# utiasSTARS/GraphIK

Measured on AMD Instinct MI355X. Metric: IK solves/sec (batched random goals), higher is better.
Workload: dtype f64

## Files before the change

graphik_amd/_ffi.py:

```python
import ctypes as C
import os

import torch

_HERE = os.path.dirname(os.path.abspath(__file__))
LIB_PATH = os.environ.get("GIK_LIB_PATH") or os.path.join(_HERE, "lib", "libgraphik_amd.so")

TERM_EQ, TERM_LOWER, TERM_UPPER = 1, 2, 3
ABI_VERSION = 10


class TemplateDesc(C.Structure):
    _fields_ = [
        ("abi_version", C.c_int32), ("N", C.c_int32), ("k", C.c_int32), ("n_terms", C.c_int32),
        ("term_i", C.POINTER(C.c_int32)), ("term_j", C.POINTER(C.c_int32)),
        ("term_kind", C.POINTER(C.c_int32)),
        ("mingradnorm", C.c_double), ("maxiter", C.c_int32), ("maxinner", C.c_int32),
        ("mininner", C.c_int32), ("theta", C.c_double), ("kappa", C.c_double),
        ("rho_prime", C.c_double), ("rho_regularization", C.c_double),
        ("planar_proj_exact", C.c_int32), ("force_block_path", C.c_int32),
        ("waves_per_cu", C.c_int32), ("slice_outer_its", C.c_int32), ("debug_flags", C.c_int32),
        ("solver", C.c_int32), ("cg_minstepsize", C.c_double), ("cg_orth_value", C.c_double),
        ("cg_beta_type", C.c_int32), ("clique_closed_form", C.c_int32), ("hessian_form", C.c_int32),
    ]


CLIQUE_AUTO, CLIQUE_OFF, CLIQUE_DENSE = 0, 1, 2
HESS_COLUMN, HESS_PER_EDGE, HESS_AUTO = 0, 1, 2


class TemplateInfo(C.Structure):
    _fields_ = [("is_block", C.c_int32), ("max_terms_per_node", C.c_int32), ("n_clique", C.c_int32),
                ("n_slot_terms", C.c_int32), ("slots_per_thread", C.c_int32), ("waves_per_cu", C.c_int32),
                ("n_cu", C.c_int32), ("lds_bytes", C.c_int32), ("clique_closed_form", C.c_int32),
                ("anchored", C.c_int32), ("has_pipeline", C.c_int32), ("prepare_is_block", C.c_int32),
                ("node_per_lane", C.c_int32), ("problems_per_wave", C.c_int32), ("goals_per_wave", C.c_int32),
                ("hessian_form", C.c_int32)]


SOLVER_TRUST_REGIONS, SOLVER_CONJUGATE_GRADIENT = 0, 1


class Stats(C.Structure):
    _fields_ = [("f", C.c_double), ("gradnorm", C.c_double), ("iterations", C.c_int32),
                ("inner_total", C.c_int32), ("stop", C.c_int32), ("n_accept", C.c_int32),
                ("inner_executed", C.c_int32), ("flags", C.c_int32), ("stepsize", C.c_double)]


STATS_BYTES = C.sizeof(Stats)
STATS_I32 = {name: getattr(Stats, name).offset // 4 for name, ct in Stats._fields_ if ct is C.c_int32}
STATS_F64 = {name: getattr(Stats, name).offset // 8 for name, ct in Stats._fields_ if ct is C.c_double}


class Trace(C.Structure):
    _fields_ = [("cap", C.c_int32), ("d_Delta", C.c_void_p), ("d_numit", C.c_void_p),
                ("d_stop", C.c_void_p), ("d_f_before", C.c_void_p),
                ("d_gradnorm_after", C.c_void_p), ("d_accept", C.c_void_p)]


class PipelineDesc(C.Structure):
# ... 65 lines not shown
                                        C.c_void_p, C.c_void_p, C.c_void_p, C.c_void_p, C.c_void_p]),
    "gik_anchored_seed_batch": (C.c_int, [C.c_void_p, C.c_void_p, C.c_void_p, C.c_void_p, C.c_int, C.c_void_p,
                                          C.c_void_p, C.c_void_p, C.c_void_p]),
    "gik_anchored_clearance": (C.c_int, [C.c_void_p, C.c_void_p, C.c_int, C.c_void_p, C.c_void_p]),
    "gik_anchored_attach_links": (C.c_int, [C.c_void_p, C.POINTER(LinkDesc)]),
    "gik_anchored_link_clearance": (C.c_int, [C.c_void_p, C.c_void_p, C.c_int, C.c_void_p, C.c_void_p]),
    "gik_anchored_sweep_ws_bytes": (C.c_size_t, [C.c_void_p, C.c_void_p, C.c_int, C.c_int]),
    "gik_anchored_sweep_clearance": (C.c_int, [C.c_void_p, C.c_void_p, C.c_void_p, C.c_void_p, C.c_int, C.c_int, C.c_void_p,
                                               C.c_void_p, C.c_void_p]),
    "gik_anchored_ik_batch_seeded": (C.c_int, [C.c_void_p, C.c_void_p, C.c_void_p, C.c_void_p, C.c_int] +
                                     7 * [C.c_void_p] + [C.c_void_p]),
    "gik_anchored_last_solve_ms": (C.c_double, [C.c_void_p]),
    "gik_anchored_retry_select": (C.c_int, [C.c_void_p, C.c_void_p, C.c_void_p, C.c_void_p, C.c_int, C.c_double,
                                            C.c_double, C.c_double, C.c_void_p, C.c_void_p, C.c_void_p]),
    "gik_anchored_retry_seeds": (C.c_int, [C.c_void_p, C.c_void_p, C.c_void_p, C.c_int, C.c_uint64, C.c_int, C.c_void_p,
                                           C.c_void_p, C.c_void_p, C.c_double, C.c_void_p, C.c_void_p, C.c_void_p]),
    "gik_anchored_retry_merge": (C.c_int, [C.c_void_p, C.c_void_p, C.c_void_p, C.c_int, C.c_int, C.c_double, C.c_double,
                                           C.c_double] + 13 * [C.c_void_p] + [C.c_void_p]),
    "gik_anchored_retry_ws_bytes": (C.c_size_t, [C.c_void_p, C.c_void_p, C.c_int]),
    "gik_anchored_ik_batch_retry": (C.c_int, [C.c_void_p, C.c_void_p, C.c_void_p, C.c_void_p, C.c_int,
                                              C.POINTER(AnchoredRetryOpts)] + 8 * [C.c_void_p] + [C.c_void_p]),
    "gik_template_destroy": (None, [C.c_void_p]),
    "gik_template_get_info": (C.c_int, [C.c_void_p, C.POINTER(TemplateInfo)]),
    "gik_cost": (C.c_int, [C.c_void_p, C.c_void_p, C.c_void_p, C.c_int, C.c_void_p, C.c_void_p]),
    "gik_grad": (C.c_int, [C.c_void_p, C.c_void_p, C.c_void_p, C.c_int, C.c_void_p, C.c_void_p]),
    "gik_cost_and_grad": (C.c_int, [C.c_void_p, C.c_void_p, C.c_void_p, C.c_int, C.c_void_p, C.c_void_p,
                                    C.c_void_p]),
    "gik_hess": (C.c_int, [C.c_void_p, C.c_void_p, C.c_void_p, C.c_void_p, C.c_int, C.c_void_p,
                           C.c_void_p]),
    "gik_proj": (C.c_int, [C.c_void_p, C.c_void_p, C.c_void_p, C.c_int, C.c_void_p, C.c_void_p]),
    "gik_solve_batch": (C.c_int, [C.c_void_p, C.c_void_p, C.c_void_p, C.c_int, C.c_void_p,
                                  C.c_void_p, C.POINTER(Trace), C.c_void_p]),
    "gik_pipeline_attach": (C.c_int, [C.c_void_p, C.POINTER(PipelineDesc)]),
    "gik_prepare_batch": (C.c_int, [C.c_void_p, C.c_void_p, C.c_int, C.c_void_p, C.c_void_p,
                                    C.c_void_p, C.c_void_p]),
    "gik_prepare_batch_debug": (C.c_int, [C.c_void_p, C.c_void_p, C.c_int, C.c_void_p, C.c_void_p,
                                          C.c_void_p, C.POINTER(PrepareDiag), C.c_void_p]),
    "gik_recover_batch": (C.c_int, [C.c_void_p, C.c_void_p, C.c_void_p, C.c_int, C.c_void_p,
                                    C.c_void_p, C.c_void_p, C.c_void_p]),
    "gik_ik_batch": (C.c_int, [C.c_void_p, C.c_void_p, C.c_int, C.c_void_p, C.c_void_p,
                               C.c_void_p, C.c_void_p, C.c_void_p, C.c_void_p, C.c_void_p]),
    "gik_seed_batch": (C.c_int, [C.c_void_p, C.c_void_p, C.c_void_p, C.c_int, C.c_void_p, C.c_void_p,
                                 C.c_void_p]),
    "gik_ik_batch_seeded": (C.c_int, [C.c_void_p, C.c_void_p, C.c_void_p, C.c_int, C.c_void_p, C.c_void_p,
                                      C.c_void_p, C.c_void_p, C.c_void_p, C.c_void_p, C.c_void_p]),
    "gik_retry_select": (C.c_int, [C.c_void_p, C.c_void_p, C.c_void_p, C.c_int, C.c_double, C.c_double,
# ... 54 lines not shown
```

graphik_amd/build.py:

```python
import glob
import hashlib
import os
import shutil
import subprocess
import sys

HERE = os.path.dirname(os.path.abspath(__file__))
REPO = os.path.dirname(HERE)
SRC = os.path.join(HERE, "csrc")
LIB = os.path.join(HERE, "lib", "libgraphik_amd.so")
DEV_LIB = os.path.join(HERE, "lib", "exp", "libgraphik_amd_dev.so")
SOURCES = ["gik_host.hip", "gik_k_wave3.hip", "gik_k_wave3_strict.hip", "gik_k_anch.hip", "gik_k_wave2.hip",
           "gik_k_block.hip", "gik_k_npt.hip", "gik_k_npt4.hip", "gik_k_quad.hip", "gik_k_prep.hip", "gik_k_retry.hip", "gik_k_anch_seed.hip",
           "gik_k_anch_retry.hip"]
FLAGS = ["--offload-arch=gfx950", "-O3", "-std=c++17", "-fPIC"]
LINK_FLAGS = ["--offload-arch=gfx950", "-shared", "-fPIC"]
UNIT_FLAGS = {"gik_k_wave3_strict.hip": ["-mllvm", "-structurizecfg-skip-uniform-regions"]}


def headers():
    return sorted(glob.glob(os.path.join(SRC, "*.h")) + glob.glob(os.path.join(REPO, "include", "*.h")))


def dependencies():
    deps = sorted(glob.glob(os.path.join(SRC, "*.hip")) + headers())
    assert all(os.path.join(SRC, s) in deps for s in SOURCES)
    return deps


def source_digest(extra=()):
    h = hashlib.sha256(" ".join(FLAGS + LINK_FLAGS + list(extra)).encode())
    h.update(repr(sorted(UNIT_FLAGS.items())).encode())
    for d in dependencies():
        h.update(os.path.relpath(d, REPO).encode())
        h.update(open(d, "rb").read())
    return h.hexdigest()

# ... 90 lines not shown
```

graphik_amd/csrc/gik_host.hip:

```cpp

#include "gik_kernels.hip.h"
#include "gik_instances.h"
#include "gik_retry.hip.h"
#include "gik_anch_seed.hip.h"
#include "gik_anch_retry.hip.h"
#include "gik_plan.h"
#include "gik_slots.h"
#include <climits>
#include <memory>

namespace gik {
GIK_ALL_KERNELS(GIK_EXTERN_TEMPLATE)
static_assert(PLAN_MIG_SIMDS == MIG_SIMDS && PLAN_SLICE_STATE_BYTES == sizeof(SliceState) && PLAN_QUAD_SLOTS == QUAD_SLOTS,
              "gik_plan.h restates these constants of the kernel headers");

struct NptVariant {
  int TL, NW;
  void (*solve)(SolveArgs);
  void (*kat)(KatArgs);
  size_t (*lds)(int, int, int, int);
  size_t (*ctg)(int);
};
#define GIK_NPT_VARIANT(TL, NS, NW, CTG) \
  {TL, NW, rtr_npt_kernel<TL, NS, NW, CTG>, kat_npt_kernel<TL, NS, NW, CTG>, NptCtx<TL, NS, NW, CTG>::lds_bytes, NptCtx<TL, NS, NW, CTG>::ctg_doubles}
static const NptVariant kNptVariants[] = {GIK_NPT_VARIANT(1, 1, 2, false), GIK_NPT_VARIANT(4, 1, 2, false),
                                          GIK_NPT_VARIANT(1, 2, 1, false), GIK_NPT_VARIANT(4, 2, 1, false),
                                          GIK_NPT_VARIANT(1, 1, 4, true),  GIK_NPT_VARIANT(4, 1, 4, true)};

thread_local std::string g_err;
#ifdef GIK_DEV
static double *g_dbg_buf = nullptr;
#endif
static int fail(const std::string &m) {
  g_err = m;
  return -1;
}
#define HIP_OK(expr)                                                                      \
// ... 69 lines not shown
  hipEvent_t ev_solve0 = nullptr, ev_solve1 = nullptr;
  gik::AnchArgs an = {};
  double *d_targets_const = nullptr;
  int full_N = 0, n_anchor = 0;
  int *d_free_full = nullptr, *d_anchor_full = nullptr;
  int *d_clear_full = nullptr;
  int n_clear = 0;
  int *d_link_a = nullptr, *d_link_b = nullptr;
  double *d_link_rho = nullptr;
  int n_link = -1;
  double axis_length = 1.0;
  int solver;
  gik::CgParams cg;
  gik::Params p;
  struct Kernels {
    void (*solve)(gik::SolveArgs) = nullptr;
    void (*solve_spread)(gik::SolveArgs) = nullptr;
    void (*kat)(gik::KatArgs) = nullptr;
    void (*block_solve)(gik::SolveArgs, int) = nullptr;
    void (*block_kat)(gik::KatArgs, int) = nullptr;
    const void *occupancy = nullptr;
  } kernels;
  uint32_t *d_slot_meta = nullptr;
  unsigned int *d_counters = nullptr;
  struct CounterSlot {
    hipEvent_t done = nullptr;
    bool pending = false;
    bool in_use = false;
  };
  std::vector<CounterSlot> counter_slot;
  unsigned next_counter = 0;
  int counter_ring = 256;
  std::mutex call_mutex;
  std::mutex ev_mutex;
  int clique_mode = 0;
  bool hess_per_edge = false;
  struct SliceWs {
    void *base = nullptr;
    size_t bytes = 0;
    hipEvent_t done = nullptr;
    bool pending = false;
    bool in_use = false;
  };
  static constexpr int kSlicePool = 32;
  SliceWs slice_ws[kSlicePool];
  unsigned next_slice = 0;
// ... 1865 lines not shown
  a.slot_meta = t->d_slot_meta;
  a.bt = t->bt;
  a.targets = d_targets;
  a.Y_init = d_Y_init;
  a.Y_out = d_Y_out;
  a.stats = d_stats;
  a.has_trace = (trace && trace->cap > 0) ? 1 : 0;
  if (a.has_trace)
    a.trace = *trace;
  else
    std::memset(&a.trace, 0, sizeof(a.trace));
  a.N = t->N;
  a.T = t->T;
  a.B = B;
  a.p = t->p;
  a.cg = t->cg;
  if (t->anchored) {
    a.an = t->an;
    a.an.anchor_goal = d_targets;
    a.targets = t->d_targets_const;
  }
  a.dbg = t->f.dbg;
  a.dbg_buf = nullptr;
#ifdef GIK_DEV
  if (a.dbg & (4 | 8 | 4096)) a.dbg_buf = dev_debug_buffer();
#endif
  a.y_head = a.y_tail = a.y_seq = nullptr;
  a.y_ids = a.y_avail = nullptr;
  a.y_cap = 0;
  a.q_tail = a.q_done = a.q_head = nullptr;
  a.mig_credits = a.mig_simd_run = nullptr;
  a.q_ids = nullptr;
  a.q_seq = nullptr;
  a.q_state = nullptr;
}

static bool event_done(hipEvent_t e) {
  if (hipEventQuery(e) == hipSuccess) return true;
  (void)hipGetLastError();
  return false;
}

typedef gik::SlotLease<gik_template::CounterSlot> CounterLease;
typedef gik::SlotLease<gik_template::SliceWs> WorkspaceLease;

static int lease_counter(gik_template *mt, CounterLease &lease, gik::SolveArgs &a, hipStream_t stream) {
  using namespace gik;
  gik_template::CounterSlot &cs = lease.take(mt->counter_slot, mt->next_counter, (unsigned)mt->counter_ring, event_done);
  a.work_counter = mt->d_counters + (&cs - mt->counter_slot.data());
  if (!cs.done && hipEventCreateWithFlags(&cs.done, hipEventDisableTiming) != hipSuccess)
    return fail("hipEventCreate failed");
  if (cs.pending) HIP_OK(hipStreamWaitEvent(stream, cs.done, 0));
  HIP_OK(hipMemsetAsync(a.work_counter, 0, sizeof(unsigned int), stream));
  return 0;
}

static int bind_workspace(gik_template *mt, WorkspaceLease &lease, const gik::SolvePlan &p, gik::SolveArgs &a,
                          hipStream_t stream) {
  using namespace gik;
  gik_template::SliceWs *sw = &lease.take(mt->slice_ws, mt->next_slice, (unsigned)mt->slice_pool, event_done);
  if (!sw->done && hipEventCreateWithFlags(&sw->done, hipEventDisableTiming) != hipSuccess)
    return fail("hipEventCreate failed");
  if (sw->bytes < p.bytes) {
    if (sw->pending) (void)hipEventSynchronize(sw->done);
    if (sw->base) (void)hipFree(sw->base);
    sw->base = nullptr;
    sw->bytes = 0;
    if (hipMalloc(&sw->base, p.bytes) != hipSuccess) return fail("cannot allocate the time-slicing workspace");
    sw->bytes = p.bytes;
    sw->pending = false;
  }
  if (sw->pending) HIP_OK(hipStreamWaitEvent(stream, sw->done, 0));
  char *base = static_cast<char *>(sw->base);
  a.q_tail = reinterpret_cast<unsigned int *>(base);
  a.q_done = a.q_tail + 1;
  a.q_head = a.q_tail + 2;
  a.mig_credits = reinterpret_cast<int *>(a.q_tail + 3);
  a.mig_simd_run = reinterpret_cast<int *>(base + p.off_simd);
  a.q_seq = reinterpret_cast<unsigned int *>(base + p.off_seq);
  a.q_ids = reinterpret_cast<int *>(base + p.off_ids);
  a.q_state = reinterpret_cast<SliceState *>(base + p.off_state);
  a.y_head = a.q_tail + 4;
  a.y_tail = a.q_tail + 5;
  a.y_avail = reinterpret_cast<int *>(a.q_tail + 6);
  a.y_seq = reinterpret_cast<unsigned int *>(base + p.off_yseq);
  a.y_ids = reinterpret_cast<int *>(base + p.off_yids);
  a.y_cap = (unsigned int)p.ycap;
  a.npt_ctg_ws = p.ctg_bytes ? reinterpret_cast<double *>(base + p.off_ctg) : nullptr;
  HIP_OK(hipMemsetAsync(base, 0, p.zero_head, stream));
  if (p.seq_fill) HIP_OK(hipMemsetAsync(a.q_seq, 0xFF, p.seq_fill, stream));
  if (p.state_zero) HIP_OK(hipMemsetAsync(a.q_state, 0, p.state_zero, stream));
  if (p.yseq_zero) HIP_OK(hipMemsetAsync(a.y_seq, 0, p.yseq_zero, stream));
  return 0;
}

static void launch(const gik_template *t, const gik::SolvePlan &p, gik::SolveArgs &a, hipStream_t stream) {
  using namespace gik;
  const dim3 grid(p.launch_grid);
  switch (p.launch) {
    case Launch::QUAD:
      hipLaunchKernelGGL(t->quad_solve, grid, dim3(WAVE), t->quad_smem, stream, a);
      break;
    case Launch::NPT:
      a.nt = t->nt;
      hipLaunchKernelGGL(t->npt_variant->solve, grid, dim3(WAVE * t->npt_variant->NW), t->npt_smem, stream, a);
      break;
    case Launch::BLOCK:
      hipLaunchKernelGGL(t->kernels.block_solve, grid, dim3(BLOCK_NT), t->smem_bytes, stream, a, t->SL);
      break;
    case Launch::WAVE:
      hipLaunchKernelGGL(t->kernels.solve, grid, dim3(WAVE), t->smem_bytes, stream, a);
      break;
    case Launch::WAVE_SPREAD:
      hipLaunchKernelGGL(t->kernels.solve_spread, grid, dim3(WAVE), t->smem_bytes, stream, a);
      break;
// ... 12 lines not shown
  fill_args(t, a, d_Y_init, d_targets, B, d_Y_out, d_stats, trace);
  if (refuse_capture("gik_solve_batch", stream_)) return -1;
  const SolvePlan plan = plan_solve(t->f, B);
  a.slice_its = plan.slice_its;
  a.slice_cycles = plan.slice_cycles;
  gik_template *mt = const_cast<gik_template *>(t);
  CounterLease counter(mt->call_mutex);
  WorkspaceLease workspace(mt->call_mutex);
  if (lease_counter(mt, counter, a, stream)) return -1;
  if (plan.needs_ws && bind_workspace(mt, workspace, plan, a, stream)) return -1;
  launch(t, plan, a, stream);
  HIP_OK(hipGetLastError());
  const hipError_t e_cs = hipEventRecord(counter.get()->done, stream);
  const hipError_t e_sw = workspace.get() ? hipEventRecord(workspace.get()->done, stream) : hipSuccess;
  if (e_cs != hipSuccess || e_sw != hipSuccess) {
    (void)hipStreamSynchronize(stream);
    return fail(std::string("hipEventRecord failed after the launch: ") + hipGetErrorString(e_cs != hipSuccess ? e_cs : e_sw));
  }
  counter.covered_by_event();
  workspace.covered_by_event();
  return 0;
}

int gik_template_get_info(const gik_template *t, gik_template_info *info) {
  if (!t || !info) return gik::fail("null argument");
  std::memset(info, 0, sizeof(*info));
  info->is_block = t->f.is_block ? 1 : 0;
  info->max_terms_per_node = t->f.is_block ? 0 : t->maxdeg;
  info->n_clique = t->bt.n_clq;
  info->n_slot_terms = t->f.is_block ? t->bt.Tc : t->T;
  info->slots_per_thread = t->SL;
  info->waves_per_cu = t->f.waves_per_cu;
  info->n_cu = t->f.n_cu;
  info->lds_bytes = (int32_t)t->smem_bytes;
  info->clique_closed_form = t->clique_mode;
  info->hessian_form = (t->hess_per_edge || t->f.is_block) ? GIK_HESS_PER_EDGE : GIK_HESS_COLUMN;
  info->anchored = t->anchored ? 1 : 0;
  info->has_pipeline = t->has_pipe ? 1 : 0;
  info->prepare_is_block = t->prep_block ? 1 : 0;
  info->node_per_lane = t->f.is_npt ? t->npt_variant->NW : 0;
  info->goals_per_wave = !t->has_pipe || t->prep_block ? 0 : (t->prep_quad ? gik::QUAD_SLOTS : 1);
  info->problems_per_wave = t->f.is_block ? 0 : ((t->quad_solve && !(t->f.dbg & (1 | 8192))) ? gik::QUAD_SLOTS : 1);
  if (t->f.is_npt) {
    info->waves_per_cu = t->f.npt_waves_per_cu;
    info->lds_bytes = (int32_t)t->npt_smem;
  }
  return 0;
}

#ifdef GIK_DEV
double gik_debug_parts(const gik_template *t, int mode, int iters) {
  using namespace gik;
  double *d = nullptr, h[2] = {0, 0};
  if (hipMalloc((void **)&d, 2 * sizeof(double)) != hipSuccess) return -1;
  hipEvent_t e0, e1;
  (void)hipEventCreate(&e0);
  (void)hipEventCreate(&e1);
  (void)hipEventRecord(e0, 0);
  if (t->f.K == 3 && t->maxdeg == 9)
    hipLaunchKernelGGL((parts_kernel<3, 9>), dim3(1), dim3(WAVE), t->smem_bytes, 0, t->d_slot_meta,
                       t->N, t->T, mode % 100, iters, d);
  else if (t->f.K == 3 && t->maxdeg == 10)
    hipLaunchKernelGGL((parts_kernel<3, 10>), dim3(1), dim3(WAVE), t->smem_bytes, 0, t->d_slot_meta,
                       t->N, t->T, mode % 100, iters, d);
// ... 22 lines not shown
```

graphik_amd/csrc/gik_kernels.hip.h:

```cpp
#pragma once
#include <hip/hip_runtime.h>

#include <algorithm>
#include <atomic>
#include <cmath>
#include <cstdio>
#include <cstring>
#include <mutex>
#include <thread>
#include <cstdlib>
#include <string>
#include <vector>

#include "gik_block.hip.h"
#include "gik_npt.hip.h"
#include "gik_quad.hip.h"
#include "gik_prep.hip.h"
#include "gik_prep_quad.hip.h"
#include "gik_rcg.hip.h"
#include "gik_rtr.hip.h"
#include "gik_rtrv.hip.h"
#include "gik_wave.hip.h"
#ifdef GIK_STRICT_HEADER
#include GIK_STRICT_HEADER
// ... 46 lines not shown
__device__ inline void requeue_work(unsigned int *q_tail, int *q_ids, unsigned int *q_seq, int B, int b) {
  const unsigned int t = atomicAdd(q_tail, 1u);
  __hip_atomic_store(&q_ids[t], b, __ATOMIC_RELAXED, __HIP_MEMORY_SCOPE_AGENT);
  __hip_atomic_store(&q_seq[t], (unsigned)B + t, __ATOMIC_RELEASE, __HIP_MEMORY_SCOPE_AGENT);
}

struct AnchArgs {
  const double *anch_const;
  const double *anchor_goal;
  const uint32_t *pin_meta;
  const double *pin_tgt;
  const double *obs;
  unsigned long long obs_mask;
  int n_obs, n_goal, goal_row0;
};

struct SolveArgs {
  const uint32_t *slot_meta;
  const double *targets;
  const double *Y_init;
  double *Y_out;
  gik_stats *stats;
  unsigned int *work_counter;
  gik_trace trace;
  int has_trace;
  int N, T, B;
  int dbg;
  double *dbg_buf;
  Params p;
  CgParams cg;
  AnchArgs an;
  int slice_its;
  int slice_cycles;
  unsigned int *q_head;
  int *mig_credits, *mig_simd_run;
  unsigned int *y_head, *y_tail, *y_seq;
  int *y_ids, *y_avail;
  unsigned int y_cap;
  unsigned int *q_tail, *q_done;
  int *q_ids;
  unsigned int *q_seq;
  SliceState *q_state;
  BlockTabs bt;
  NptTabs nt;
  double *npt_ctg_ws = nullptr;
};
// ... 121 lines not shown
              if (__hip_atomic_load(a.y_avail, __ATOMIC_RELAXED, __HIP_MEMORY_SCOPE_AGENT) > 0) {
                if (__hip_atomic_fetch_add(a.y_avail, -1, __ATOMIC_ACQUIRE, __HIP_MEMORY_SCOPE_AGENT) > 0) {
                  pop = true;
                  break;
                }
                __hip_atomic_fetch_add(a.y_avail, 1, __ATOMIC_RELAXED, __HIP_MEMORY_SCOPE_AGENT);
              }
              b = mig_wait(mig, a.q_head, a.q_seq, a.q_ids, a.q_done, a.B);
              if (b != -2) break;
            }
            if (pop) {
              const unsigned int h = __hip_atomic_fetch_add(a.y_head, 1u, __ATOMIC_RELAXED, __HIP_MEMORY_SCOPE_AGENT);
              while (__hip_atomic_load(&a.y_seq[h], __ATOMIC_ACQUIRE, __HIP_MEMORY_SCOPE_AGENT) != h + 1u)
                __builtin_amdgcn_s_sleep(2);
              b = __hip_atomic_load(&a.y_ids[h], __ATOMIC_RELAXED, __HIP_MEMORY_SCOPE_AGENT);
              __hip_atomic_fetch_add(&mig.simd_run[mig.sid], 1, __ATOMIC_RELAXED, __HIP_MEMORY_SCOPE_AGENT);
            }
          }
          owns_entry = false;
        }
        b = __builtin_amdgcn_readlane(b, 0);
        resumed = __builtin_amdgcn_readlane(resumed, 0);
      }
      tail = tail || resumed;
#ifdef GIK_DEV
      dev_t_claim += (long long)__builtin_readcyclecounter() - dev_tc;
      ++dev_n_claim;
      if ((a.dbg & 4096) && a.dbg_buf && lane == 0) dev_log(a.dbg_buf, resumed ? 1 : 0, b);
#endif
      if (UNI(b < 0)) break;
    } else {
      if (a.dbg & 1) {
        b = (int)blockIdx.x + pass * (int)gridDim.x;
        ++pass;
      } else {
        if (lane == 0) b = (int)atomicAdd(a.work_counter, 1u);
        b = __builtin_amdgcn_readlane(b, 0);
      }
      if (UNI(b >= a.B)) break;
    }

    if constexpr (ANCH) {
      if (lane < 3 * a.an.n_goal)
        cx.sh_anch[(a.an.goal_row0 + lane / 3) * 4 + lane % 3] =
            a.an.anchor_goal[(size_t)b * 3 * a.an.n_goal + lane];
      cx.obs_reset();
    } else {
      for (int t = lane; t < a.T; t += WAVE) sh_tgt[t] = a.targets[(size_t)b * a.T + t];
      __builtin_amdgcn_wave_barrier();
      cx.load_slot_records();
    }
    RtrOut ro;
    double x;
    int rs_resumes = 0;
    if constexpr (MIG) {
      RtrResume rs = load_slice_state(&a.q_state[b]);
      rs.resumed = resumed;
      rs_resumes = rs.resumes;
      const double *src = resumed ? a.Y_out : a.Y_init;
// ... 913 lines not shown
```

graphik_amd/csrc/gik_plan.h:

```cpp
#pragma once

#include <algorithm>
#include <cstddef>

namespace gik {

constexpr int PLAN_MIG_SIMDS = 1 << 14;
constexpr size_t PLAN_SLICE_STATE_BYTES = 32;
constexpr int PLAN_QUAD_SLOTS = 4;

struct SolveFacts {
  int K = 0;
  bool is_block = false;
  bool is_npt = false;
  bool cg = false;
  int n_cu = 0;
  int waves_per_cu = 0;
  int npt_waves_per_cu = 1;
  int wpc_override = 0;
  int slice_its = 0;
  int npt_slice_its = 192;
  int maxiter = 0;
  int dbg = 0;
  bool has_spread = false;
  int wave_slice_its = 0;
  bool wave_slice_auto = true;
  int wave_slice_cycles = 2000000;
  bool has_quad = false;
  int quad_min_batch = -1;
  int quad_waves_per_cu = 8;
  size_t ctg_doubles = 0;
};

enum class Launch { QUAD, NPT, BLOCK, WAVE, WAVE_SPREAD };

struct SolvePlan {
  Launch launch;
  int grid;
  int launch_grid;
  int wpc;
  int slice_its, slice_cycles;
  bool mig;
  size_t cap, ycap;
  bool needs_ws;
  size_t off_simd, off_seq, off_ids, off_state, off_yseq, off_yids, off_ctg, bytes;
  size_t ctg_bytes;
  size_t zero_head, seq_fill, state_zero, yseq_zero;
};

inline SolvePlan plan_solve(const SolveFacts &t, int B) {
  SolvePlan p = {};
  int wpc = t.is_npt ? t.npt_waves_per_cu : t.waves_per_cu;
  if (!t.is_block && t.K == 3 && wpc > 4 && (long long)B <= 6LL * 4 * t.n_cu) wpc = 4;
  if (!t.is_block && t.K == 3 && wpc > 8 && (long long)B < 128LL * t.n_cu) wpc = 8;
  if (t.wpc_override > 0) wpc = t.wpc_override;
  const int grid = std::min(B, t.n_cu * wpc);
  int slice = t.is_npt ? t.npt_slice_its : t.slice_its;
  if (!t.is_block || t.cg || B <= grid || (t.dbg & 1) || slice <= 0 || t.maxiter <= slice) slice = 0;
  const bool mig = t.has_spread && wpc > 4 && B > grid && !(t.dbg & (1 | 512));
  const size_t ctg_bytes = t.is_npt ? t.ctg_doubles * sizeof(double) * (size_t)grid : 0;
  p.wpc = wpc;
  p.grid = p.launch_grid = grid;
  p.slice_its = slice;
  p.mig = mig;
  p.needs_ws = slice > 0 || mig || ctg_bytes;
  if (p.needs_ws) {
    const size_t cap = mig ? (size_t)B + (size_t)grid + 64 : (slice > 0 ? (size_t)B * (size_t)(t.maxiter / slice + 1) : 0);
    int wslice = (mig && !(t.dbg & 1024)) ? t.wave_slice_its : 0;
    if (wslice > 0 && t.wave_slice_auto && (long long)B > 8LL * grid)
      wslice = (int)std::min<long long>(4LL * wslice, (long long)wslice * B / (8LL * grid));
    const size_t ycap = wslice > 0 ? std::min((size_t)B * (size_t)(t.maxiter / wslice + 2), (size_t)16 * B + 8192) +
                                         2 * (size_t)grid + 256
                                   : 0;
    const size_t off_simd = 32, off_seq = off_simd + (mig ? sizeof(int) * PLAN_MIG_SIMDS : 0), off_ids = off_seq + cap * 4,
                 off_state = (off_ids + cap * 4 + 15) & ~(size_t)15,
                 off_yseq = off_state + (((size_t)B * PLAN_SLICE_STATE_BYTES + 15) & ~(size_t)15), off_yids = off_yseq + ycap * 4;
    const size_t off_ctg = (off_yids + ycap * 4 + 63) & ~(size_t)63;
    const size_t bytes = off_ctg + ctg_bytes;
    if (mig) { p.slice_its = wslice; p.slice_cycles = t.wave_slice_cycles; }
    p.cap = cap;
    p.ycap = ycap;
    p.off_simd = off_simd;
    p.off_seq = off_seq;
    p.off_ids = off_ids;
    p.off_state = off_state;
    p.off_yseq = off_yseq;
    p.off_yids = off_yids;
    p.off_ctg = off_ctg;
    p.ctg_bytes = ctg_bytes;
    p.bytes = bytes;
    p.zero_head = off_seq;
    p.seq_fill = cap * 4;
    p.state_zero = (mig || t.is_npt) ? (size_t)B * PLAN_SLICE_STATE_BYTES : 0;
    p.yseq_zero = ycap * 4;
  }
  const bool quad = t.has_quad && !(t.dbg & (1 | 8192)) && ((t.dbg & 16384) || B >= t.quad_min_batch);
  if (quad) {
    int qw = t.quad_waves_per_cu;
    if (t.wpc_override > 0) qw = t.wpc_override;
    p.launch_grid = std::max(1, std::min((B + PLAN_QUAD_SLOTS - 1) / PLAN_QUAD_SLOTS, t.n_cu * qw));
    p.launch = Launch::QUAD;
  } else if (t.is_npt) {
    p.launch = Launch::NPT;
  } else if (t.is_block) {
    p.launch = Launch::BLOCK;
  } else {
    p.launch = mig ? Launch::WAVE_SPREAD : Launch::WAVE;
  }
  return p;
}

}
```

graphik_amd/engine.py:

```python
import ctypes as C

import numpy as np
import torch

from . import _ffi


def build_terms(omega, psi_L=None, psi_U=None, use_limits=True):
    omega = np.asarray(omega, dtype=float)
    N = omega.shape[0]
    if use_limits:
        psi_L = np.asarray(psi_L, dtype=float)
        psi_U = np.asarray(psi_U, dtype=float)
        diff = psi_L != psi_U
        inds = np.nonzero(np.triu(omega) + np.triu(diff * (psi_L > 0)) + np.triu(diff * (psi_U > 0)))
    else:
        psi_L = np.zeros((N, N))
        psi_U = np.zeros((N, N))
        inds = np.nonzero(np.triu(omega))
    ti, tj, tk, tv = [], [], [], []
    for i, j in zip(*inds):
        if omega[i, j] != 0:
            ti.append(i); tj.append(j); tk.append(_ffi.TERM_EQ); tv.append(np.nan)
        if psi_L[i, j] != 0:
# ... 62 lines not shown
        raise ValueError("clearance_mode='links' needs a link set: this problem was built without links")
    return _ffi.CLEARANCE_MODES[clearance_mode]


class Template:

    def __init__(self, N, k, term_i, term_j, term_kind, targets_static=None, device=None,
                 params=None, anchored=None):
        self.lib = _ffi.lib()
        if not torch.cuda.is_available():
            raise _ffi.GikError("no HIP device visible: graphik_amd needs an AMD GPU (gfx950)")
        self.device = torch.device(device if device is not None else
                                   f"cuda:{torch.cuda.current_device()}")
        self.N, self.k = int(N), int(k)
        self.term_i = np.ascontiguousarray(term_i, dtype=np.int32)
        self.term_j = np.ascontiguousarray(term_j, dtype=np.int32)
        self.term_kind = np.ascontiguousarray(term_kind, dtype=np.int32)
        self.T = len(self.term_i)
        self.targets_static = None if targets_static is None else \
            np.ascontiguousarray(targets_static, dtype=np.float64)
        d = _ffi.TemplateDesc()
        params = dict(params or {})
        self.solver = params.pop("solver", "TrustRegions")
        if self.solver == "ConjugateGradient":
            self.lib.gik_default_cg_params(C.byref(d))
        elif self.solver == "TrustRegions":
            self.lib.gik_default_params(C.byref(d))
        else:
            raise ValueError("params[\"solver\"] must be one of 'ConjugateGradient', 'TrustRegions'")
        d.N, d.k, d.n_terms = self.N, self.k, self.T
        d.term_i = self.term_i.ctypes.data_as(C.POINTER(C.c_int32))
        d.term_j = self.term_j.ctypes.data_as(C.POINTER(C.c_int32))
        d.term_kind = self.term_kind.ctypes.data_as(C.POINTER(C.c_int32))
        alias = {"minstepsize": "cg_minstepsize", "orth_value": "cg_orth_value", "beta_type": "cg_beta_type"}
        for key, val in params.items():
            key = alias.get(key, key)
            if not hasattr(d, key):
                raise KeyError(f"unknown solver parameter {key!r}")
            if key == "clique_closed_form" and isinstance(val, str):
                val = {"auto": _ffi.CLIQUE_AUTO, "off": _ffi.CLIQUE_OFF, "dense": _ffi.CLIQUE_DENSE}[val]
            if key == "hessian_form" and isinstance(val, str):
                val = {"column": _ffi.HESS_COLUMN, "per_edge": _ffi.HESS_PER_EDGE, "auto": _ffi.HESS_AUTO}[val]
            setattr(d, key, int(val) if key in ("maxiter", "cg_beta_type", "clique_closed_form", "hessian_form") else val)
        self.params = {f: getattr(d, f) for f in ("mingradnorm", "maxiter", "maxinner", "mininner",
                                                   "theta", "kappa", "rho_prime",
                                                   "rho_regularization", "planar_proj_exact",
# ... 33 lines not shown
        self._h = h
        self.n_link = None
        self._read_info()
        deg = np.bincount(np.concatenate([self.term_i, self.term_j]), minlength=self.N).max()
        self.maxdeg = int(self.info["max_terms_per_node"]) if not self.info["is_block"] else int(deg)

    def _read_info(self):
        info = _ffi.TemplateInfo()
        _ffi.check(self.lib.gik_template_get_info(self._h, C.byref(info)))
        self.info = {f: getattr(info, f) for f, _ in _ffi.TemplateInfo._fields_ if f != "reserved"}

    @classmethod
    def from_matrices(cls, omega, psi_L=None, psi_U=None, k=3, use_limits=True, **kw):
        ti, tj, tk, tv = build_terms(omega, psi_L, psi_U, use_limits)
        return cls(np.asarray(omega).shape[0], k, ti, tj, tk, tv, **kw)

    def __del__(self):
        try:
            if getattr(self, "_h", None):
                self.lib.gik_template_destroy(self._h)
                self._h = None
        except Exception:
            pass

    def targets_from_D(self, D_goal):
        D = np.asarray(D_goal, dtype=np.float64)
        if D.ndim == 2:
            D = D[None]
        tg = D[:, self.term_i, self.term_j].copy()
        if self.targets_static is not None:
            hinge = self.term_kind != _ffi.TERM_EQ
            tg[:, hinge] = self.targets_static[hinge]
        return tg

    def _stream(self):
        return C.c_void_p(torch.cuda.current_stream(self.device).cuda_stream)

    def _vec(self, Y):
        Y = _dev(Y, self.device)
        if Y.dim() == 2:
            Y = Y[None]
        B = Y.shape[0]
        return Y.reshape(B, self.N * self.k).contiguous(), B

    def _tg(self, targets, B):
        t = _dev(targets, self.device)
# ... 406 lines not shown
```

graphik_amd/solvers/riemannian_solver.py:

```python
import collections
import hashlib
import time

import numpy as np
import torch

from ..engine import Template, _alloc_stats, _decode_stats, build_terms, check_clearance_mode, check_retry_args
from ..utils import dgp
from ..utils.constants import POS
from ..utils.lie import as_matrix

_STOP_REASONS = {0: "Terminated - min grad norm reached", 1: "Terminated - max iterations reached",
                 2: "Terminated - NaN encountered", 3: "Terminated - min stepsize reached"}
BetaTypes = ["FletcherReeves", "PolakRibiere", "HestenesStiefel", "HagerZhang"]


_closure_templates = collections.OrderedDict()
_CLOSURE_TEMPLATES_MAX = 8


def _cost_closures(D_goal, omega, psi_L, psi_U, use_limits):
    omega = np.asarray(omega, dtype=float)
    psi_L = None if psi_L is None else np.asarray(psi_L, dtype=float)
    psi_U = None if psi_U is None else np.asarray(psi_U, dtype=float)
# ... 146 lines not shown
                                                                            graph.index(e)]))
        self.anchor_nodes = [i for i, name in enumerate(graph.node_ids)
                             if POS in graph.nodes[name] and i not in self.goal_nodes]
        self.anchor_pos = np.array([graph.nodes[graph.node_ids[i]][POS] for i in self.anchor_nodes],
                                   dtype=float)
        q0 = self.robot.zero_configuration()
        G0 = graph.from_pose({e: self.robot.pose(q0, e) for e in self.end_effectors})
        self.omega = dgp.adjacency_matrix_from_graph(G0)
        self.base_D = dgp.distance_matrix_from_graph(G0)
        self.base_lower = np.where(G0.edge, G0.lower, np.nan)
        self.base_upper = np.where(G0.edge, G0.upper, np.nan)
        if use_limits:
            self.psi_L, self.psi_U = graph.distance_bound_matrices()
        else:
            self.psi_L = self.psi_U = None
        self.N = N
        self.terms = build_terms(self.omega, self.psi_L, self.psi_U, use_limits)
        if host_only:
            self.template, self.device_pipeline = None, False
            return
        self.template = Template.from_matrices(self.omega, self.psi_L, self.psi_U, k=self.dim,
                                               use_limits=use_limits, device=device, params=params)
        self._attach_device_pipeline()

    def _attach_device_pipeline(self):
        g, T = self.graph, self.template
        n = self.robot.n
        if len(self.anchor_nodes) > 256 or self.N > (255 if self.dim == 3 else 128) or len(self.end_effectors) > 8:
            self.device_pipeline = False
            return
        if self.dim == 3:
            dev_slots = list(self.goal_nodes)
        else:
            dev_slots, seen = [], set()
            for e in self.end_effectors:
                for name in (e, self.robot.parent[e]):
                    node = g.index(name)
                    dev_slots.append(node if node not in seen else -1)
                    seen.add(node)
            if any(dev_slots[2 * e] < 0 for e in range(len(self.end_effectors))):
                self.device_pipeline = False
                return
        goal_slot = {node: sl for sl, node in enumerate(dev_slots) if node >= 0}
        goalset = set(self.goal_nodes)
        slot = {a: s for s, a in enumerate(self.anchor_nodes)}
        G = len(dev_slots)
# ... 682 lines not shown
```

graphik_amd/utils/roboturdf.py:

```python
import json
import os
import xml.etree.ElementTree as ET

import numpy as np

from ..graphs import ProblemGraphRevolute
from ..robots import RobotRevolute
from ..utils.lie import SE3

_DATA = os.path.join(os.path.dirname(os.path.dirname(os.path.abspath(__file__))), "data", "robots")


def _packaged(name):
    with open(os.path.join(_DATA, name + ".json")) as f:
        rec = json.load(f)
    T = np.array([[[float.fromhex(v) for v in row] for row in M] for M in rec["T_zero"]])
    return rec["num_joints"], T


def _randomize_links(T, pct):
    T = [np.array(M, dtype=float) for M in T]
    for idx in range(len(T) - 1):
        D = np.linalg.inv(T[idx]) @ T[idx + 1]
        t = D[:3, 3] * ((1 - pct) + 2 * pct * np.random.rand())
        t[np.abs(t) < 1e-6] = 0
        D[:3, 3] = t
        T[idx + 1] = T[idx] @ D
    return np.array(T)


def _make(n, T_zero, limits, randomized_links=False, randomize_percentage=0.4):
    if randomized_links:
        T_zero = _randomize_links(T_zero, randomize_percentage)
    if limits is None:
        ub = np.ones(n) * np.pi
        lb = -ub
    else:
        lb, ub = limits[0], limits[1]
    params = {"T_zero": {f"p{i}": T_zero[i] for i in range(n + 1)}, "num_joints": n,
              "joint_limits_upper": list(ub), "joint_limits_lower": list(lb),
              "parents": {f"p{i}": ([f"p{i + 1}"] if i < n else []) for i in range(n + 1)}}
    robot = RobotRevolute(params)
    return robot, ProblemGraphRevolute(robot)


def load_schunk_lwa4d(limits=None, randomized_links=False, randomize_percentage=0.4):
    return _make(*_packaged("lwa4d"), limits, randomized_links, randomize_percentage)


def load_ur10(limits=None, randomized_links=False, randomize_percentage=0.4):
    return _make(*_packaged("ur10"), limits, randomized_links, randomize_percentage)


def load_kuka(limits=None, randomized_links=False, randomize_percentage=0.4):
    return _make(*_packaged("kuka"), limits, randomized_links, randomize_percentage)


def load_schunk_lwa4p(limits=None, randomized_links=False, randomize_percentage=0.4):
    return _make(*_packaged("lwa4p"), limits, randomized_links, randomize_percentage)


def load_panda(limits=None, randomized_links=False, randomize_percentage=0.4):
    return _make(*_packaged("panda"), limits, randomized_links, randomize_percentage)


def load_truncated_ur10(n):
    a = [0, -0.612, -0.5723, 0, 0, 0][:n]
    d = [0.1273, 0, 0, 0.1639, 0.1157, 0.0922][:n]
    al = [np.pi / 2, 0, 0, np.pi / 2, -np.pi / 2, 0][:n]
    params = {"a": a, "alpha": al, "d": d, "theta": [0] * n, "modified_dh": False,
# ... 93 lines not shown
```

include/graphik_amd.h:

```cpp
#ifndef GRAPHIK_AMD_H
#define GRAPHIK_AMD_H

#include <stdint.h>

#ifdef __cplusplus
extern "C" {
#endif

#define GIK_ABI_VERSION 10

enum { GIK_TERM_EQ = 1, GIK_TERM_LOWER = 2, GIK_TERM_UPPER = 3 };

typedef struct {
  int32_t abi_version;
  int32_t N;
  int32_t k;
  int32_t n_terms;
  const int32_t *term_i;
  const int32_t *term_j;
  const int32_t *term_kind;
  double mingradnorm;
  int32_t maxiter;
  int32_t maxinner;
  int32_t mininner;
  double theta;
  double kappa;
  double rho_prime;
  double rho_regularization;
  int32_t planar_proj_exact;
  int32_t force_block_path;
  int32_t waves_per_cu;
  int32_t slice_outer_its;
// ... 45 lines not shown
void gik_default_params(gik_template_desc *desc);
void gik_default_cg_params(gik_template_desc *desc);

int gik_template_create(const gik_template_desc *desc, gik_template **out);
void gik_template_destroy(gik_template *t);

typedef struct {
  int32_t is_block;
  int32_t max_terms_per_node;
  int32_t n_clique;
  int32_t n_slot_terms;
  int32_t slots_per_thread;
  int32_t waves_per_cu;
  int32_t n_cu;
  int32_t lds_bytes;
  int32_t clique_closed_form;
  int32_t anchored;
  int32_t has_pipeline;
  int32_t prepare_is_block;
  int32_t node_per_lane;
  int32_t problems_per_wave;
  int32_t goals_per_wave;
  int32_t hessian_form;
} gik_template_info;
int gik_template_get_info(const gik_template *t, gik_template_info *info);

int gik_cost(const gik_template *t, const double *d_Y, const double *d_targets, int B,
             double *d_f, void *stream);
int gik_grad(const gik_template *t, const double *d_Y, const double *d_targets, int B,
             double *d_out, void *stream);
int gik_cost_and_grad(const gik_template *t, const double *d_Y, const double *d_targets, int B,
                      double *d_f, double *d_grad, void *stream);
int gik_hess(const gik_template *t, const double *d_Y, const double *d_W,
             const double *d_targets, int B, double *d_out, void *stream);
int gik_proj(const gik_template *t, const double *d_Y, const double *d_Z, int B,
             double *d_out, void *stream);

int gik_solve_batch(const gik_template *t, const double *d_Y_init, const double *d_targets,
                    int B, double *d_Y_out, gik_stats *d_stats, const gik_trace *trace,
                    void *stream);

typedef struct {
  int32_t n_joints;
  const double *T0;
  const int32_t *p_index;
  const int32_t *q_index;
  int32_t x_index, y_index;
  double axis_length;
// ... 170 lines not shown
```

Before: 38700.

## Order dynamic work claims by a goal-reach key to balance batch tails

Adds a per-problem key computed from selected target distance terms (e.g., base-to-goal distances), ranks problems with a new counting-sort kernel, and makes the dynamic work-claim loop pick problems in that sorted order. The intent is to group problems of similar difficulty or iteration count so waves finish together and the long tail at the end of the batch shrinks. It costs two extra small kernel launches plus an O(B^2) rank kernel per solve, and an extra indirection per claim. It is enabled automatically only for robots whose packaged data declares a 'reach' claim key (lwa4d).

```diff
diff --git a/graphik_amd/_ffi.py b/graphik_amd/_ffi.py
--- a/graphik_amd/_ffi.py
+++ b/graphik_amd/_ffi.py
@@ -7,7 +7,7 @@
 LIB_PATH = os.environ.get("GIK_LIB_PATH") or os.path.join(_HERE, "lib", "libgraphik_amd.so")
 
 TERM_EQ, TERM_LOWER, TERM_UPPER = 1, 2, 3
-ABI_VERSION = 10
+ABI_VERSION = 11
 
 
 class TemplateDesc(C.Structure):
@@ -35,7 +35,7 @@
                 ("n_cu", C.c_int32), ("lds_bytes", C.c_int32), ("clique_closed_form", C.c_int32),
                 ("anchored", C.c_int32), ("has_pipeline", C.c_int32), ("prepare_is_block", C.c_int32),
                 ("node_per_lane", C.c_int32), ("problems_per_wave", C.c_int32), ("goals_per_wave", C.c_int32),
-                ("hessian_form", C.c_int32)]
+                ("hessian_form", C.c_int32), ("claim_key_terms", C.c_int32)]
 
 
 SOLVER_TRUST_REGIONS, SOLVER_CONJUGATE_GRADIENT = 0, 1
@@ -147,6 +147,10 @@
                                               C.POINTER(AnchoredRetryOpts)] + 8 * [C.c_void_p] + [C.c_void_p]),
     "gik_template_destroy": (None, [C.c_void_p]),
     "gik_template_get_info": (C.c_int, [C.c_void_p, C.POINTER(TemplateInfo)]),
+    "gik_template_set_claim_key": (C.c_int, [C.c_void_p, C.c_int, C.POINTER(C.c_int32), C.POINTER(C.c_double)]),
+    "gik_claim_order_max_batch": (C.c_int, []),
+    "gik_claim_order_keys": (C.c_int, [C.c_void_p, C.c_void_p, C.c_int, C.c_void_p, C.c_void_p]),
+    "gik_claim_order_sort": (C.c_int, [C.c_void_p, C.c_int, C.c_void_p, C.c_void_p]),
     "gik_cost": (C.c_int, [C.c_void_p, C.c_void_p, C.c_void_p, C.c_int, C.c_void_p, C.c_void_p]),
     "gik_grad": (C.c_int, [C.c_void_p, C.c_void_p, C.c_void_p, C.c_int, C.c_void_p, C.c_void_p]),
     "gik_cost_and_grad": (C.c_int, [C.c_void_p, C.c_void_p, C.c_void_p, C.c_int, C.c_void_p, C.c_void_p,
diff --git a/graphik_amd/build.py b/graphik_amd/build.py
--- a/graphik_amd/build.py
+++ b/graphik_amd/build.py
@@ -12,7 +12,7 @@
 DEV_LIB = os.path.join(HERE, "lib", "exp", "libgraphik_amd_dev.so")
 SOURCES = ["gik_host.hip", "gik_k_wave3.hip", "gik_k_wave3_strict.hip", "gik_k_anch.hip", "gik_k_wave2.hip",
            "gik_k_block.hip", "gik_k_npt.hip", "gik_k_npt4.hip", "gik_k_quad.hip", "gik_k_prep.hip", "gik_k_retry.hip", "gik_k_anch_seed.hip",
-           "gik_k_anch_retry.hip"]
+           "gik_k_anch_retry.hip", "gik_k_order.hip"]
 FLAGS = ["--offload-arch=gfx950", "-O3", "-std=c++17", "-fPIC"]
 LINK_FLAGS = ["--offload-arch=gfx950", "-shared", "-fPIC"]
 UNIT_FLAGS = {"gik_k_wave3_strict.hip": ["-mllvm", "-structurizecfg-skip-uniform-regions"]}
diff --git a/graphik_amd/csrc/gik_host.hip b/graphik_amd/csrc/gik_host.hip
--- a/graphik_amd/csrc/gik_host.hip
+++ b/graphik_amd/csrc/gik_host.hip
@@ -4,6 +4,7 @@
 #include "gik_retry.hip.h"
 #include "gik_anch_seed.hip.h"
 #include "gik_anch_retry.hip.h"
+#include "gik_order.hip.h"
 #include "gik_plan.h"
 #include "gik_slots.h"
 #include <climits>
@@ -13,6 +14,7 @@
 GIK_ALL_KERNELS(GIK_EXTERN_TEMPLATE)
 static_assert(PLAN_MIG_SIMDS == MIG_SIMDS && PLAN_SLICE_STATE_BYTES == sizeof(SliceState) && PLAN_QUAD_SLOTS == QUAD_SLOTS,
               "gik_plan.h restates these constants of the kernel headers");
+static_assert(PLAN_CLAIM_KEY_MAX_TERMS == CLAIM_KEY_MAX_TERMS, "gik_plan.h restates this constant of gik_order.hip.h");
 
 struct NptVariant {
   int TL, NW;
@@ -128,6 +130,7 @@
     const void *occupancy = nullptr;
   } kernels;
   uint32_t *d_slot_meta = nullptr;
+  gik::ClaimKey claim_key;
   unsigned int *d_counters = nullptr;
   struct CounterSlot {
     hipEvent_t done = nullptr;
@@ -2039,6 +2042,7 @@
   }
   a.dbg = t->f.dbg;
   a.dbg_buf = nullptr;
+  a.claim_order = nullptr;
 #ifdef GIK_DEV
   if (a.dbg & (4 | 8 | 4096)) a.dbg_buf = dev_debug_buffer();
 #endif
@@ -2070,6 +2074,13 @@
   if (cs.pending) HIP_OK(hipStreamWaitEvent(stream, cs.done, 0));
   HIP_OK(hipMemsetAsync(a.work_counter, 0, sizeof(unsigned int), stream));
   return 0;
+}
+
+static void launch_claim_order(const gik::ClaimKey &k, const double *d_targets, int T, int B, float *d_key, int *d_order,
+                               hipStream_t stream) {
+  using namespace gik;
+  if (d_targets) hipLaunchKernelGGL(claim_key_kernel, dim3((B + 255) / 256), dim3(256), 0, stream, d_targets, T, B, k, d_key);
+  hipLaunchKernelGGL(claim_rank_kernel, dim3((B + ORDER_ROWS - 1) / ORDER_ROWS), dim3(ORDER_NT), 0, stream, d_key, B, d_order);
 }
 
 static int bind_workspace(gik_template *mt, WorkspaceLease &lease, const gik::SolvePlan &p, gik::SolveArgs &a,
@@ -2104,10 +2115,17 @@
   a.y_ids = reinterpret_cast<int *>(base + p.off_yids);
   a.y_cap = (unsigned int)p.ycap;
   a.npt_ctg_ws = p.ctg_bytes ? reinterpret_cast<double *>(base + p.off_ctg) : nullptr;
-  HIP_OK(hipMemsetAsync(base, 0, p.zero_head, stream));
+  if (p.zero_head) HIP_OK(hipMemsetAsync(base, 0, p.zero_head, stream));
   if (p.seq_fill) HIP_OK(hipMemsetAsync(a.q_seq, 0xFF, p.seq_fill, stream));
   if (p.state_zero) HIP_OK(hipMemsetAsync(a.q_state, 0, p.state_zero, stream));
   if (p.yseq_zero) HIP_OK(hipMemsetAsync(a.y_seq, 0, p.yseq_zero, stream));
+  if (p.order) {
+    float *key = reinterpret_cast<float *>(base + p.off_key);
+    int *order = reinterpret_cast<int *>(base + p.off_order);
+    launch_claim_order(mt->claim_key, a.targets, a.T, a.B, key, order, stream);
+    HIP_OK(hipGetLastError());
+    a.claim_order = order;
+  }
   return 0;
 }
 
@@ -2166,6 +2184,52 @@
   return 0;
 }
 
+int gik_template_set_claim_key(gik_template *t, int n, const int32_t *terms, const double *weights) {
+  using namespace gik;
+  if (!t) return fail("null argument");
+  if (n > 0 && !weights) return fail("claim key: weights required");
+  if (!claim_key_ok(n, terms, t->T))
+    return fail("claim key: at most " + std::to_string(PLAN_CLAIM_KEY_MAX_TERMS) + " terms, each an index into the template's " +
+                std::to_string(t->T) + " terms");
+  if (t->anchored || t->f.is_block || t->f.K != 3 || t->f.cg) n = 0;
+  if (const char *e = getenv("GIK_CLAIM_ORDER"))
+    if (!std::strcmp(e, "off") || !std::strcmp(e, "0")) n = 0;
+  ClaimKey k;
+  k.n = n;
+  for (int i = 0; i < n; ++i) {
+    k.term[i] = terms[i];
+    k.w[i] = weights[i];
+  }
+  std::lock_guard<std::mutex> lock(t->call_mutex);
+  t->claim_key = k;
+  t->f.claim_terms = n;
+  return 0;
+}
+
+int gik_claim_order_max_batch(void) { return gik::PLAN_CLAIM_ORDER_MAX_BATCH; }
+
+int gik_claim_order_keys(const gik_template *t, const double *d_targets, int B, float *d_keys, void *stream) {
+  using namespace gik;
+  if (!t || B < 0) return fail("bad argument");
+  if (t->claim_key.n == 0) return fail("the template has no claim key");
+  if (B == 0) return 0;
+  if (!d_targets || !d_keys) return fail("null buffer");
+  hipLaunchKernelGGL(claim_key_kernel, dim3((B + 255) / 256), dim3(256), 0, (hipStream_t)stream, d_targets, t->T, B,
+                     t->claim_key, d_keys);
+  HIP_OK(hipGetLastError());
+  return 0;
+}
+
+int gik_claim_order_sort(const float *d_keys, int B, int32_t *d_order, void *stream) {
+  using namespace gik;
+  if (B < 0 || B > PLAN_CLAIM_ORDER_MAX_BATCH) return fail("claim order: 0 .. " + std::to_string(PLAN_CLAIM_ORDER_MAX_BATCH) + " keys");
+  if (B == 0) return 0;
+  if (!d_keys || !d_order) return fail("null buffer");
+  launch_claim_order(ClaimKey(), nullptr, 0, B, const_cast<float *>(d_keys), d_order, (hipStream_t)stream);
+  HIP_OK(hipGetLastError());
+  return 0;
+}
+
 int gik_template_get_info(const gik_template *t, gik_template_info *info) {
   if (!t || !info) return gik::fail("null argument");
   std::memset(info, 0, sizeof(*info));
@@ -2184,6 +2248,7 @@
   info->prepare_is_block = t->prep_block ? 1 : 0;
   info->node_per_lane = t->f.is_npt ? t->npt_variant->NW : 0;
   info->goals_per_wave = !t->has_pipe || t->prep_block ? 0 : (t->prep_quad ? gik::QUAD_SLOTS : 1);
+  info->claim_key_terms = t->f.claim_terms;
   info->problems_per_wave = t->f.is_block ? 0 : ((t->quad_solve && !(t->f.dbg & (1 | 8192))) ? gik::QUAD_SLOTS : 1);
   if (t->f.is_npt) {
     info->waves_per_cu = t->f.npt_waves_per_cu;
diff --git a/graphik_amd/csrc/gik_k_order.hip b/graphik_amd/csrc/gik_k_order.hip
--- /dev/null
+++ b/graphik_amd/csrc/gik_k_order.hip
@@ -0,0 +1,2 @@
+#define GIK_DEFINE_ORDER_KERNELS 1
+#include "gik_order.hip.h"
diff --git a/graphik_amd/csrc/gik_kernels.hip.h b/graphik_amd/csrc/gik_kernels.hip.h
--- a/graphik_amd/csrc/gik_kernels.hip.h
+++ b/graphik_amd/csrc/gik_kernels.hip.h
@@ -92,6 +92,7 @@
   double *Y_out;
   gik_stats *stats;
   unsigned int *work_counter;
+  const int *claim_order = nullptr;
   gik_trace trace;
   int has_trace;
   int N, T, B;
@@ -259,6 +260,7 @@
         b = __builtin_amdgcn_readlane(b, 0);
         resumed = __builtin_amdgcn_readlane(resumed, 0);
       }
+      if (a.claim_order && !resumed && b >= 0) b = a.claim_order[b];
       tail = tail || resumed;
 #ifdef GIK_DEV
       dev_t_claim += (long long)__builtin_readcyclecounter() - dev_tc;
@@ -270,8 +272,12 @@
       if (a.dbg & 1) {
         b = (int)blockIdx.x + pass * (int)gridDim.x;
         ++pass;
+        if (a.claim_order && b < a.B) b = a.claim_order[b];
       } else {
-        if (lane == 0) b = (int)atomicAdd(a.work_counter, 1u);
+        if (lane == 0) {
+          b = (int)atomicAdd(a.work_counter, 1u);
+          if (a.claim_order && b < a.B) b = a.claim_order[b];
+        }
         b = __builtin_amdgcn_readlane(b, 0);
       }
       if (UNI(b >= a.B)) break;
diff --git a/graphik_amd/csrc/gik_order.hip.h b/graphik_amd/csrc/gik_order.hip.h
--- /dev/null
+++ b/graphik_amd/csrc/gik_order.hip.h
@@ -0,0 +1,64 @@
+#pragma once
+
+#include <hip/hip_runtime.h>
+#include <stdint.h>
+
+namespace gik {
+
+constexpr int CLAIM_KEY_MAX_TERMS = 8;
+constexpr int ORDER_ROWS = 64;
+constexpr int ORDER_PARTS = 4;
+constexpr int ORDER_NT = ORDER_ROWS * ORDER_PARTS;
+constexpr int ORDER_TILE = 1024;
+
+struct ClaimKey {
+  int n = 0;
+  int term[CLAIM_KEY_MAX_TERMS] = {};
+  double w[CLAIM_KEY_MAX_TERMS] = {};
+};
+
+__host__ __device__ inline uint32_t claim_key_code(float k) {
+  if (k != k) return 0xffffffffu;
+  union { float f; uint32_t u; } v;
+  v.f = k == 0.0f ? 0.0f : k;
+  return (v.u & 0x80000000u) ? ~v.u : (v.u | 0x80000000u);
+}
+
+#ifdef GIK_DEFINE_ORDER_KERNELS
+__global__ void __launch_bounds__(256) claim_key_kernel(const double *targets, int T, int B, ClaimKey k, float *key) {
+  const int b = (int)(blockIdx.x * blockDim.x + threadIdx.x);
+  if (b >= B) return;
+  double s = 0.0;
+  for (int i = 0; i < k.n; ++i) s += k.w[i] * targets[(size_t)b * T + k.term[i]];
+  key[b] = (float)s;
+}
+
+__global__ void __launch_bounds__(ORDER_NT) claim_rank_kernel(const float *key, int B, int *order) {
+  __shared__ uint32_t sh_code[ORDER_TILE];
+  __shared__ int sh_cnt[ORDER_PARTS][ORDER_ROWS];
+  const int row = (int)threadIdx.x % ORDER_ROWS, part = (int)threadIdx.x / ORDER_ROWS;
+  const int i = (int)blockIdx.x * ORDER_ROWS + row;
+  const uint64_t mine = i < B ? ((uint64_t)claim_key_code(key[i]) << 32) | (uint32_t)i : 0;
+  int cnt = 0;
+  for (int j0 = 0; j0 < B; j0 += ORDER_TILE) {
+    const int n = min(ORDER_TILE, B - j0);
+    __syncthreads();
+    for (int j = (int)threadIdx.x; j < n; j += ORDER_NT) sh_code[j] = claim_key_code(key[j0 + j]);
+    __syncthreads();
+    const int q = (n + ORDER_PARTS - 1) / ORDER_PARTS, lo = part * q, hi = min(n, lo + q);
+    for (int j = lo; j < hi; ++j) cnt += ((((uint64_t)sh_code[j] << 32) | (uint32_t)(j0 + j)) < mine) ? 1 : 0;
+  }
+  sh_cnt[part][row] = cnt;
+  __syncthreads();
+  if (part == 0 && i < B) {
+    int pos = 0;
+    for (int p = 0; p < ORDER_PARTS; ++p) pos += sh_cnt[p][row];
+    order[pos] = i;
+  }
+}
+#else
+__global__ void claim_key_kernel(const double *targets, int T, int B, ClaimKey k, float *key);
+__global__ void claim_rank_kernel(const float *key, int B, int *order);
+#endif
+
+}
diff --git a/graphik_amd/csrc/gik_plan.h b/graphik_amd/csrc/gik_plan.h
--- a/graphik_amd/csrc/gik_plan.h
+++ b/graphik_amd/csrc/gik_plan.h
@@ -8,6 +8,15 @@
 constexpr int PLAN_MIG_SIMDS = 1 << 14;
 constexpr size_t PLAN_SLICE_STATE_BYTES = 32;
 constexpr int PLAN_QUAD_SLOTS = 4;
+constexpr int PLAN_CLAIM_KEY_MAX_TERMS = 8;
+constexpr int PLAN_CLAIM_ORDER_MAX_BATCH = 65536;
+
+inline bool claim_key_ok(int n, const int *terms, int T) {
+  if (n < 0 || n > PLAN_CLAIM_KEY_MAX_TERMS || (n > 0 && !terms)) return false;
+  for (int i = 0; i < n; ++i)
+    if (terms[i] < 0 || terms[i] >= T) return false;
+  return true;
+}
 
 struct SolveFacts {
   int K = 0;
@@ -30,6 +39,7 @@
   int quad_min_batch = -1;
   int quad_waves_per_cu = 8;
   size_t ctg_doubles = 0;
+  int claim_terms = 0;
 };
 
 enum class Launch { QUAD, NPT, BLOCK, WAVE, WAVE_SPREAD };
@@ -42,10 +52,12 @@
   int slice_its, slice_cycles;
   bool mig;
   size_t cap, ycap;
+  bool order;
   bool needs_ws;
   size_t off_simd, off_seq, off_ids, off_state, off_yseq, off_yids, off_ctg, bytes;
   size_t ctg_bytes;
   size_t zero_head, seq_fill, state_zero, yseq_zero;
+  size_t off_key, off_order;
 };
 
 inline SolvePlan plan_solve(const SolveFacts &t, int B) {
@@ -63,7 +75,9 @@
   p.grid = p.launch_grid = grid;
   p.slice_its = slice;
   p.mig = mig;
-  p.needs_ws = slice > 0 || mig || ctg_bytes;
+  p.order = t.claim_terms > 0 && !t.is_block && !t.is_npt && t.K == 3 && !t.cg && B > grid && B <= PLAN_CLAIM_ORDER_MAX_BATCH;
+  const bool queues = slice > 0 || mig || ctg_bytes;
+  p.needs_ws = queues || p.order;
   if (p.needs_ws) {
     const size_t cap = mig ? (size_t)B + (size_t)grid + 64 : (slice > 0 ? (size_t)B * (size_t)(t.maxiter / slice + 1) : 0);
     int wslice = (mig && !(t.dbg & 1024)) ? t.wave_slice_its : 0;
@@ -76,7 +90,8 @@
                  off_state = (off_ids + cap * 4 + 15) & ~(size_t)15,
                  off_yseq = off_state + (((size_t)B * PLAN_SLICE_STATE_BYTES + 15) & ~(size_t)15), off_yids = off_yseq + ycap * 4;
     const size_t off_ctg = (off_yids + ycap * 4 + 63) & ~(size_t)63;
-    const size_t bytes = off_ctg + ctg_bytes;
+    const size_t off_key = (off_ctg + ctg_bytes + 63) & ~(size_t)63, off_order = off_key + (p.order ? 4 * (size_t)B : 0);
+    const size_t bytes = p.order ? off_order + 4 * (size_t)B : off_ctg + ctg_bytes;
     if (mig) { p.slice_its = wslice; p.slice_cycles = t.wave_slice_cycles; }
     p.cap = cap;
     p.ycap = ycap;
@@ -89,7 +104,9 @@
     p.off_ctg = off_ctg;
     p.ctg_bytes = ctg_bytes;
     p.bytes = bytes;
-    p.zero_head = off_seq;
+    p.off_key = off_key;
+    p.off_order = off_order;
+    p.zero_head = queues ? off_seq : 0;
     p.seq_fill = cap * 4;
     p.state_zero = (mig || t.is_npt) ? (size_t)B * PLAN_SLICE_STATE_BYTES : 0;
     p.yseq_zero = ycap * 4;
diff --git a/graphik_amd/engine.py b/graphik_amd/engine.py
--- a/graphik_amd/engine.py
+++ b/graphik_amd/engine.py
@@ -108,6 +108,9 @@
         d = _ffi.TemplateDesc()
         params = dict(params or {})
         self.solver = params.pop("solver", "TrustRegions")
+        self.claim_order = params.pop("claim_order", "auto")
+        if self.claim_order not in ("auto", "on", "off"):
+            raise ValueError("params[\"claim_order\"] must be one of 'auto', 'on', 'off'")
         if self.solver == "ConjugateGradient":
             self.lib.gik_default_cg_params(C.byref(d))
         elif self.solver == "TrustRegions":
@@ -187,6 +190,31 @@
                 self._h = None
         except Exception:
             pass
+
+    def set_claim_key(self, terms, weights):
+        terms = np.ascontiguousarray(terms, dtype=np.int32).reshape(-1)
+        w = np.ascontiguousarray(weights, dtype=np.float64).reshape(-1)
+        if len(terms) != len(w):
+            raise ValueError("one weight per term")
+        n = 0 if self.claim_order == "off" else len(terms)
+        with torch.cuda.device(self.device):
+            _ffi.check(self.lib.gik_template_set_claim_key(self._h, n, terms.ctypes.data_as(C.POINTER(C.c_int32)),
+                                                           w.ctypes.data_as(C.POINTER(C.c_double))))
+        self._read_info()
+
+    def claim_order_of(self, keys):
+        k = torch.as_tensor(keys, dtype=torch.float32).to(self.device).contiguous()
+        order = torch.full((k.numel(),), -1, dtype=torch.int32, device=self.device)
+        with torch.cuda.device(self.device):
+            _ffi.check(self.lib.gik_claim_order_sort(k.data_ptr(), k.numel(), order.data_ptr(), self._stream()))
+        return order
+
+    def claim_keys(self, targets):
+        t = _dev(targets, self.device)
+        keys = torch.empty(t.shape[0], dtype=torch.float32, device=self.device)
+        with torch.cuda.device(self.device):
+            _ffi.check(self.lib.gik_claim_order_keys(self._h, t.data_ptr(), t.shape[0], keys.data_ptr(), self._stream()))
+        return keys
 
     def targets_from_D(self, D_goal):
         D = np.asarray(D_goal, dtype=np.float64)
diff --git a/graphik_amd/solvers/riemannian_solver.py b/graphik_amd/solvers/riemannian_solver.py
--- a/graphik_amd/solvers/riemannian_solver.py
+++ b/graphik_amd/solvers/riemannian_solver.py
@@ -192,6 +192,20 @@
         self.template = Template.from_matrices(self.omega, self.psi_L, self.psi_U, k=self.dim,
                                                use_limits=use_limits, device=device, params=params)
         self._attach_device_pipeline()
+        mode = (params or {}).get("claim_order", "auto")
+        if mode == "on" or (mode == "auto" and getattr(self.robot, "claim_key", None) == "reach"):
+            terms = self.claim_key_terms()
+            if terms:
+                self.template.set_claim_key(terms, np.ones(len(terms)))
+
+    def claim_key_nodes(self):
+        return list(self.goal_nodes[0::2]) if self.dim == 3 else []
+
+    def claim_key_terms(self):
+        ti, tj, tk, _ = self.terms
+        p0 = self.graph.index("p0")
+        pairs = {(min(p0, g), max(p0, g)) for g in self.claim_key_nodes()}
+        return [t for t in range(len(ti)) if tk[t] == 1 and (int(ti[t]), int(tj[t])) in pairs]
 
     def _attach_device_pipeline(self):
         g, T = self.graph, self.template
diff --git a/graphik_amd/utils/roboturdf.py b/graphik_amd/utils/roboturdf.py
--- a/graphik_amd/utils/roboturdf.py
+++ b/graphik_amd/utils/roboturdf.py
@@ -44,8 +44,16 @@
     return robot, ProblemGraphRevolute(robot)
 
 
+def _claim_key(name):
+    with open(os.path.join(_DATA, name + ".json")) as f:
+        return json.load(f).get("claim_key")
+
+
 def load_schunk_lwa4d(limits=None, randomized_links=False, randomize_percentage=0.4):
-    return _make(*_packaged("lwa4d"), limits, randomized_links, randomize_percentage)
+    robot, graph = _make(*_packaged("lwa4d"), limits, randomized_links, randomize_percentage)
+    if not randomized_links:
+        robot.claim_key = _claim_key("lwa4d")
+    return robot, graph
 
 
 def load_ur10(limits=None, randomized_links=False, randomize_percentage=0.4):
diff --git a/include/graphik_amd.h b/include/graphik_amd.h
--- a/include/graphik_amd.h
+++ b/include/graphik_amd.h
@@ -7,7 +7,7 @@
 extern "C" {
 #endif
 
-#define GIK_ABI_VERSION 10
+#define GIK_ABI_VERSION 11
 
 enum { GIK_TERM_EQ = 1, GIK_TERM_LOWER = 2, GIK_TERM_UPPER = 3 };
 
@@ -99,8 +99,14 @@
   int32_t problems_per_wave;
   int32_t goals_per_wave;
   int32_t hessian_form;
+  int32_t claim_key_terms;
 } gik_template_info;
 int gik_template_get_info(const gik_template *t, gik_template_info *info);
+
+int gik_template_set_claim_key(gik_template *t, int n, const int32_t *terms, const double *weights);
+int gik_claim_order_max_batch(void);
+int gik_claim_order_keys(const gik_template *t, const double *d_targets, int B, float *d_keys, void *stream);
+int gik_claim_order_sort(const float *d_keys, int B, int32_t *d_order, void *stream);
 
 int gik_cost(const gik_template *t, const double *d_Y, const double *d_targets, int B,
              double *d_f, void *stream);
```

New measurement: 42520 (median of 6 runs). 9.9% higher.
